# StefanHeng/ECG-Representation-Learning

Hardware: AMD Instinct MI355X
Metric: 12-lead ECG records/sec pre-train step, ViT-Base bf16 @ 1/2/4/8 MI355X (higher is better)
Workload: dtype bf16

## Files before the change

### ecg-representation-learning_amd/csrc/gemm.hip

```cpp
#include "gemm_plan.h"
#include <algorithm>

namespace {

bool is_f8(int t) { return t == ECGVIT_FP8_E4M3 || t == ECGVIT_BF8_E5M2; }
bool al16(const void *p) { return reinterpret_cast<uintptr_t>(p) % 16 == 0; }
bool abc_al16(const ecgvit_gemm_desc *d) { return al16(d->A) && al16(d->B) && al16(d->C); }
bool fits31(int64_t v) { return v < (1ll << 31); }
int ceil_div(int64_t a, int b) { return (int)((a + b - 1) / b); }

bool aux_res_ok(const ecgvit_gemm_desc *d) {
    if ((d->epilogue & (ECGVIT_EPI_GELU | ECGVIT_EPI_GELU_BWD | ECGVIT_EPI_MUL_AUX)) && (!d->aux || d->ldaux % 8 || !al16(d->aux))) return false;
    return !(d->epilogue & ECGVIT_EPI_RESIDUAL) || (d->residual && d->ldr % 8 == 0 && al16(d->residual));
}

template <typename Go> auto with_nt_sets(const ecgvit_gemm_desc *d, Go &&go) {
    if (d->dtype == ECGVIT_FP8_E4M3) return go(epi_sets::E4m3{});
    if (d->dtype == ECGVIT_BF8_E5M2) return go(epi_sets::E5m2{});
    return d->out_dtype == ECGVIT_BF16 ? go(epi_sets::Bf16{}) : go(epi_sets::F32Out{});
}
bool nt_own_body(const ecgvit_gemm_desc *d) { return with_nt_sets(d, [&](auto sets) { return epi_in(sets, d->epilogue); }); }

bool nt_ok(const ecgvit_gemm_desc *d) {
    const bool f8 = is_f8(d->dtype);
// ... 16 lines not shown
    if ((epi & ECGVIT_EPI_COLSUM) &&
        (d->out_dtype != ECGVIT_BF16 || !d->workspace || !d->colsum_out || d->workspace_bytes < (int64_t)8 * ceil_div(d->M, GEMM_NT_TILE) * d->N))
        return false;
    return true;
}

bool wgrad_ok(const ecgvit_gemm_desc *d) {
    const bool f8 = is_f8(d->dtype);
    if (d->layout != ECGVIT_GEMM_TN || !(d->dtype == ECGVIT_BF16 || f8) || d->batch1 != 1 || d->batch2 != 1) return false;
    if (d->epilogue & ~(ECGVIT_EPI_BIAS | ECGVIT_EPI_ACCUM)) return false;
    if (d->K < 4096 || d->M % 256 != 0 || d->N % 256 != 0) return false;
    const int es = f8 ? 1 : 2;
    if (f8 && (d->out_dtype != ECGVIT_F32 || d->lda % 16 || d->ldb % 16 || !d->A || !d->B || !al16(d->A) || !al16(d->B)))
        return false;
    return fits31((int64_t)d->K * d->lda * es + 65536 * d->lda) && fits31((int64_t)d->K * d->ldb * es + 65536 * d->ldb);
}

int choose_splits(const ecgvit_gemm_desc *d, int ntile) {
    if (d->layout != ECGVIT_GEMM_TN) return 1;
    const int ksteps = ceil_div(d->K, GEMM_BK);
    int s = (768 + ntile - 1) / ntile;
    s = std::min(s, std::max(1, ksteps / 8));
    return std::max(1, std::min(s, 64));
}

int choose_splits2(const ecgvit_gemm_desc *d, int ntile) {
    if (d->layout != ECGVIT_GEMM_TN) return 1;
    const int ksteps = ceil_div(d->K, GEMM_BK);
    int s = 256 / ntile;
    if (s >= 8 && (s & ~7) * ntile * 100 >= s * ntile * 93) s &= ~7;
    if (s < 1) s = 1;
    s = std::min(s, std::max(1, ksteps / 16));
    return std::max(1, std::min(s, 64));
}

int64_t slab_bytes(const ecgvit_gemm_desc *d, int splits) { return splits > 1 ? (int64_t)splits * d->M * d->N * 4 : 0; }
int wgrad_splits(const ecgvit_gemm_desc *d) { return choose_splits2(d, (d->M / GEMM_WGRAD_TILE) * (d->N / GEMM_WGRAD_TILE)); }
int fit_splits(const ecgvit_gemm_desc *d, int sp) {
    while (sp > 1 && slab_bytes(d, sp) > d->workspace_bytes) --sp;
    return sp;
}

int64_t preferred_workspace(const ecgvit_gemm_desc *d) {
    const int64_t w2 = wgrad_ok(d) ? slab_bytes(d, wgrad_splits(d)) : 0;
    if (is_f8(d->dtype) && d->layout == ECGVIT_GEMM_TN) return w2;
    if (d->dtype != ECGVIT_BF16 || d->layout != ECGVIT_GEMM_TN) return 0;
// ... 67 lines not shown
}

void plan_wgrad(GemmPlan &p, const ecgvit_gemm_desc *d) {
    p.body = is_f8(d->dtype) ? GemmBody::WGRAD8 : GemmBody::WGRAD;
    p.tiles_m = d->M / GEMM_WGRAD_TILE;
    p.tiles_n = d->N / GEMM_WGRAD_TILE;
    const int ksteps = ceil_div(d->K, GEMM_BK);
    p.k_per_split = ksteps * GEMM_BK;
    const int sp = d->workspace ? fit_splits(d, wgrad_splits(d)) : 1;
    if (sp > 1) {
        p.splits = sp;
        p.k_per_split = ((ksteps + sp - 1) / sp) * GEMM_BK;
        if (is_f8(d->dtype)) p.k_per_split = ((ceil_div(d->K, 128) + sp - 1) / sp) * 128;
    }
    p.grid = dim3((unsigned)(p.tiles_m * p.tiles_n * p.splits));
}

void plan_bf16(GemmPlan &p, const ecgvit_gemm_desc *d) {
    p.body = GemmBody::BF16;
    p.tiles_m = ceil_div(d->M, GEMM_BF16_TILE);
    p.tiles_n = ceil_div(d->N, GEMM_BF16_TILE);
    const int ntile = p.tiles_m * p.tiles_n, ksteps = ceil_div(d->K, GEMM_BK);
    p.k_per_split = ksteps * GEMM_BK;
    if (d->workspace && d->layout == ECGVIT_GEMM_TN) {
        const int sp = fit_splits(d, choose_splits(d, ntile));
        if (sp > 1 && ((int64_t)d->M * d->N) % 4 == 0 && !(d->epilogue & ~(ECGVIT_EPI_BIAS | ECGVIT_EPI_ACCUM))) {
            p.splits = sp;
            p.k_per_split = ((ksteps + sp - 1) / sp) * GEMM_BK;
        }
    }
    p.grid = dim3((unsigned)(ntile * p.splits));
}

GemmPlan plan_gemm(const ecgvit_gemm_desc *d, int mask_row_pitch) {
    GemmPlan p;
    if (!d) return p;
    p.workspace = preferred_workspace(d);
    if (mask_row_pitch < 1 || (int64_t)d->N * mask_row_pitch >= (1ll << 31)) return p;
    p.mask_row_pitch = mask_row_pitch;
    const int epi = d->epilogue;
    if ((epi & (ECGVIT_EPI_NO_OUT | ECGVIT_EPI_AUX8)) && !nt_ok(d)) return p;
    if ((epi & ECGVIT_EPI_DROPOUT) && d->dropout_p > 0.f && d->out_dtype == ECGVIT_BF16 && dropout_threshold8(d->dropout_p) == 0u)
        return p;
    ecgvit_gemm_desc g = *d;
    if (epi & ECGVIT_EPI_COLSUM) {
        if (!d->colsum_out || !d->workspace || d->batch1 != 1 || d->batch2 != 1) return p;
        if (!nt_ok(d)) {
            if (!colsum_args_ok(d)) return p;
            g.epilogue &= ~ECGVIT_EPI_COLSUM;
            p.colsum = true;
        }
// ... 22 lines not shown
    switch (p.body) {
        case GemmBody::F32: rc = gemm_f32_launch(p, &g, s); break;
        case GemmBody::BF16: rc = gemm_bf16_launch(p, &g, s); break;
        case GemmBody::NT:
        case GemmBody::NT4W: rc = gemm_nt_launch(p, &g, s); break;
        default: rc = gemm_wgrad_launch(p, &g, s); break;
    }
    if (rc != ECGVIT_OK || !p.colsum) return rc;
    return ecgvit_colsum(d->C, d->ldc, d->colsum_out, d->workspace, d->M, d->N, d->out_dtype, stream);
}

}

extern "C" int ecgvit_gemm(const ecgvit_gemm_desc *d, void *stream) { return run_gemm(plan_gemm(d, 1), d, stream); }

extern "C" int ecgvit_gemm_rowpitch(const ecgvit_gemm_desc *d, int mask_row_pitch, void *stream) {
    return run_gemm(plan_gemm(d, mask_row_pitch), d, stream);
}

extern "C" int ecgvit_gemm_kernel(const ecgvit_gemm_desc *d) { return plan_gemm(d, 1).kernel; }

extern "C" int64_t ecgvit_gemm_workspace(const ecgvit_gemm_desc *d) { return plan_gemm(d, 1).workspace; }

#ifdef ECGVIT_TOOLS
extern "C" int ecgvit_tools_gemm(const ecgvit_gemm_desc *d, void *stream, int kernel, int raster_g) {
    if (kernel != 2 && kernel != 3) return ecgvit_gemm(d, stream);
    GemmPlan p = plan_gemm(d, 1);
    if (p.kernel != ECGVIT_KERNEL_GEMM_NT) return ECGVIT_EINVAL;
    if (raster_g > 0) p.group = std::min(raster_g, p.tiles_n);
    if (kernel == 3) {
        if (d->dtype != ECGVIT_BF16 || d->out_dtype != ECGVIT_BF16 || d->alpha != 1.f || d->scale_a || d->scale_b ||
            !epi_in(epi_sets::FourWave{}, d->epilogue))
            return ECGVIT_EINVAL;
        p.body = GemmBody::NT4W;
        p.fl = d->epilogue;
        p.nt_stores = false;
    }
    return run_gemm(p, d, stream);
}
#endif
```

### ecg-representation-learning_amd/csrc/gemm_bf16.hip

```cpp
#include "gemm_plan.h"
#include <cstdlib>

namespace {

constexpr int BM = GEMM_BF16_TILE, BN = GEMM_BF16_TILE, BK = GEMM_BK;
constexpr int KC_TILE_BYTES = BM * BK * 2;
constexpr int MN_ROW_BYTES = 320;
constexpr int MN_TILE_BYTES = BK * MN_ROW_BYTES;
constexpr int CS_LD = BN + 4;
constexpr int CS_BYTES = BM * CS_LD * 4;

template <bool KC> struct TileBytes { static constexpr int value = KC ? KC_TILE_BYTES : MN_TILE_BYTES; };

__device__ __forceinline__ int kc_off(int row, int chunk) { return row * 128 + ((chunk ^ ((row >> 1) & 7)) << 4); }

template <bool KC>
__device__ __forceinline__ void g_load(const bf16_t *__restrict__ P, int64_t ld, int mn0, int k0, int MN, int K, u32x4 (&r)[4]) {
    const int t = threadIdx.x;
#pragma unroll
    for (int i = 0; i < 4; ++i) {
        const int c = t + 256 * i;
        if (KC) {
            int row = mn0 + (c >> 3);
            row = row < MN ? row : MN - 1;
// ... 25 lines not shown
template <bool KC> __device__ __forceinline__ bf16x8 frag_load(const char *S, int mn_base, int ks, int lane) {
    if constexpr (KC) {
        const int row = mn_base + (lane & 31);
        return *reinterpret_cast<const bf16x8 *>(S + kc_off(row, ks * 2 + (lane >> 5)));
    } else {
        const int g = lane >> 4, i = lane & 15;
        const int col = mn_base + (g & 1) * 16 + (i & 3) * 4;
        const int k = ks * 16 + (g >> 1) * 8 + (i >> 2);
        const char *p = S + k * MN_ROW_BYTES + col * 2;
        const bf16x4 lo = __builtin_amdgcn_ds_read_tr16_b64_v4bf16((lds_bf16x4 *)(p));
        const bf16x4 hi = __builtin_amdgcn_ds_read_tr16_b64_v4bf16((lds_bf16x4 *)(p + 4 * MN_ROW_BYTES));
        const u32x2 ul = __builtin_bit_cast(u32x2, lo), uh = __builtin_bit_cast(u32x2, hi);
        u32x4 u;
        u[0] = ul[0]; u[1] = ul[1]; u[2] = uh[0]; u[3] = uh[1];
        return __builtin_bit_cast(bf16x8, u);
    }
}

__device__ __forceinline__ int xcd_remap(int bid, int nblk) {
    const int q = nblk >> 3, r = nblk & 7, x = bid & 7, j = bid >> 3;
    return (x < r ? x * (q + 1) : r * (q + 1) + (x - r) * q) + j;
}

struct SplitK {
    int splits;
    int k_per_split;
    float *slabs;
};

template <bool A_KC, bool B_KC, typename TO>
__global__ __launch_bounds__(256, 2) void gemm_bf16_kernel(ecgvit_gemm_desc d, EpiParams e, SplitK sk, int tiles_m, int tiles_n) {
    constexpr int SA = TileBytes<A_KC>::value, SB = TileBytes<B_KC>::value;
    constexpr int STAGE = SA + SB;
    constexpr int LDS_BYTES = (2 * STAGE > CS_BYTES) ? 2 * STAGE : CS_BYTES;
    __shared__ __attribute__((aligned(16))) char smem[LDS_BYTES];

    const int ntile = tiles_m * tiles_n;
    const int split = blockIdx.x / ntile;
    const int tid = xcd_remap(blockIdx.x - split * ntile, ntile);
    const int tm = tid / tiles_n, tn = tid - tm * tiles_n;
    const int m0 = tm * BM, n0 = tn * BN;
    const int M = d.M, N = d.N;
    const int kbeg = split * sk.k_per_split;
    const int kend = min(d.K, kbeg + sk.k_per_split);

    const bf16_t *A = reinterpret_cast<const bf16_t *>(d.A);
// ... 56 lines not shown
#pragma unroll
                for (int r = 0; r < 16; ++r)
                    Cs[(wm * 64 + i * 32 + (r & 3) + 8 * (r >> 2) + 4 * lh) * CS_LD + wn * 64 + j * 32 + lr] = acc[i][j][r];
    }
    __syncthreads();
    const int cc = (threadIdx.x & 15) * 8;
    const int n = n0 + cc;
#pragma unroll 2
    for (int p = 0; p < 8; ++p) {
        const int rr = p * 16 + (threadIdx.x >> 4);
        const int64_t m = m0 + rr;
        if (m >= M || n >= N) continue;
        float v[8];
        const f32x4 c0 = *reinterpret_cast<const f32x4 *>(&Cs[rr * CS_LD + cc]);
        const f32x4 c1 = *reinterpret_cast<const f32x4 *>(&Cs[rr * CS_LD + cc + 4]);
#pragma unroll
        for (int k = 0; k < 4; ++k) { v[k] = c0[k]; v[4 + k] = c1[k]; }
        if (sk.splits > 1) {
            float *o = sk.slabs + ((int64_t)split * M + m) * N + n;
            *reinterpret_cast<f32x4 *>(o) = c0;
            *reinterpret_cast<f32x4 *>(o + 4) = c1;
            continue;
        }
#pragma unroll
        for (int k = 0; k < 8; ++k) v[k] *= e.alpha;
        if (e.flags & ECGVIT_EPI_BIAS) {
            const f32x4 b0 = *reinterpret_cast<const f32x4 *>(e.bias + n), b1 = *reinterpret_cast<const f32x4 *>(e.bias + n + 4);
#pragma unroll
            for (int k = 0; k < 4; ++k) { v[k] += b0[k]; v[4 + k] += b1[k]; }
        }
        if constexpr (sizeof(TO) == 2) {
            float mult[8];
            const bool drop = e.flags & ECGVIT_EPI_DROPOUT;
            if (drop) dropout_mask8(e.seed, (uint32_t)m * (uint32_t)e.N + (uint32_t)n, e.drop_thresh, e.inv_keep, mult);
            if (e.flags & ECGVIT_EPI_GELU) {
                Vec16<bf16_t> sav;
                if (e.flags & ECGVIT_EPI_GELU_GRAD_AUX) {
#pragma unroll
                    for (int k = 0; k < 8; ++k) {
                        float dy;
                        gelu_fast_both(v[k], v[k], dy);
                        sav.set(k, drop ? dy * mult[k] : dy);
                    }
                } else {
#pragma unroll
                    for (int k = 0; k < 8; ++k) sav.set(k, v[k]);
#pragma unroll
                    for (int k = 0; k < 8; ++k) v[k] = gelu_fast(sav.get(k));
                }
                st16(reinterpret_cast<bf16_t *>(e.aux) + m * e.ldaux + n, sav);
            }
            if (drop) {
#pragma unroll
                for (int k = 0; k < 8; ++k) v[k] *= mult[k];
            }
            if (e.flags & ECGVIT_EPI_GELU_BWD) {
                const Vec16<bf16_t> pre = ld16(reinterpret_cast<const bf16_t *>(e.aux) + m * e.ldaux + n);
#pragma unroll
                for (int k = 0; k < 8; ++k) v[k] *= gelu_fast_grad(pre.get(k));
            }
            if (e.flags & ECGVIT_EPI_MUL_AUX) {
                const Vec16<bf16_t> a = ld16(reinterpret_cast<const bf16_t *>(e.aux) + m * e.ldaux + n);
#pragma unroll
                for (int k = 0; k < 8; ++k) v[k] *= a.get(k);
            }
            if (e.flags & ECGVIT_EPI_RESIDUAL) {
                const Vec16<bf16_t> res = ld16(reinterpret_cast<const bf16_t *>(e.residual) + m * e.ldr + n);
#pragma unroll
                for (int k = 0; k < 8; ++k) v[k] += res.get(k);
            }
            bf16_t *o = reinterpret_cast<bf16_t *>(d.C) + m * d.ldc + n;
            if (e.flags & ECGVIT_EPI_ACCUM) {
                const Vec16<bf16_t> old = ld16(o);
#pragma unroll
                for (int k = 0; k < 8; ++k) v[k] += old.get(k);
            }
            Vec16<bf16_t> out;
#pragma unroll
            for (int k = 0; k < 8; ++k) out.set(k, v[k]);
            st16(o, out);
        } else {
            float *o = reinterpret_cast<float *>(d.C) + m * d.ldc + n;
            if (e.flags & ECGVIT_EPI_ACCUM) {
                const f32x4 o0 = *reinterpret_cast<const f32x4 *>(o), o1 = *reinterpret_cast<const f32x4 *>(o + 4);
#pragma unroll
                for (int k = 0; k < 4; ++k) { v[k] += o0[k]; v[4 + k] += o1[k]; }
            }
            f32x4 w0, w1;
#pragma unroll
            for (int k = 0; k < 4; ++k) { w0[k] = v[k]; w1[k] = v[4 + k]; }
            *reinterpret_cast<f32x4 *>(o) = w0;
            *reinterpret_cast<f32x4 *>(o + 4) = w1;
        }
    }
}

template <typename TO>
__global__ __launch_bounds__(256) void splitk_reduce_kernel(const float *__restrict__ slabs, int splits, int64_t MN, int N,
                                                            TO *__restrict__ C, int64_t ldc, EpiParams e) {
    const int64_t nv = MN / 4;
    for (int64_t i = blockIdx.x * 256ll + threadIdx.x; i < nv; i += (int64_t)gridDim.x * 256) {
        f32x4 s = *reinterpret_cast<const f32x4 *>(slabs + i * 4);
        for (int k = 1; k < splits; ++k) s += *reinterpret_cast<const f32x4 *>(slabs + (int64_t)k * MN + i * 4);
        const int64_t m = (i * 4) / N;
        const int n = (int)((i * 4) - m * N);
        TO *o = C + m * ldc + n;
#pragma unroll
        for (int k = 0; k < 4; ++k) {
            float v = s[k] * e.alpha;
            if (e.flags & ECGVIT_EPI_BIAS) v += e.bias[n + k];
            if (e.flags & ECGVIT_EPI_ACCUM) v += to_f32<TO>(o[k]);
            o[k] = from_f32<TO>(v);
        }
    }
}

}

int gemm_bf16_launch(const GemmPlan &p, const ecgvit_gemm_desc *d, hipStream_t s) {
    SplitK sk;
    sk.splits = p.splits;
    sk.k_per_split = p.k_per_split;
    sk.slabs = p.splits > 1 ? reinterpret_cast<float *>(d->workspace) : nullptr;
    const EpiParams e = make_epi(d, p.mask_row_pitch);
#define LAUNCH(AK, BKC, TO) hipLaunchKernelGGL((gemm_bf16_kernel<AK, BKC, TO>), p.grid, dim3(256), 0, s, *d, e, sk, p.tiles_m, p.tiles_n)
    const bool obf = d->out_dtype == ECGVIT_BF16;
    switch (d->layout) {
        case ECGVIT_GEMM_NT: if (obf) LAUNCH(true, true, bf16_t); else LAUNCH(true, true, float); break;
        case ECGVIT_GEMM_NN: if (obf) LAUNCH(true, false, bf16_t); else LAUNCH(true, false, float); break;
        default: if (obf) LAUNCH(false, false, bf16_t); else LAUNCH(false, false, float); break;
    }
#undef LAUNCH
    ECGVIT_CHECK_LAUNCH();
    if (sk.splits > 1) {
        const int64_t MN = (int64_t)d->M * d->N;
        const int g = (int)std::min<int64_t>((MN / 4 + 255) / 256, 2048);
        if (obf) hipLaunchKernelGGL(splitk_reduce_kernel<bf16_t>, dim3(g), dim3(256), 0, s, sk.slabs, sk.splits, MN, d->N, (bf16_t *)d->C, d->ldc, e);
        else hipLaunchKernelGGL(splitk_reduce_kernel<float>, dim3(g), dim3(256), 0, s, sk.slabs, sk.splits, MN, d->N, (float *)d->C, d->ldc, e);
        ECGVIT_CHECK_LAUNCH();
    }
    return ECGVIT_OK;
}
```

### ecg-representation-learning_amd/csrc/gemm_plan.h

```cpp
#pragma once
#include "common.h"
#include <type_traits>

constexpr int GEMM_F32_TILE = 128, GEMM_BF16_TILE = 128, GEMM_NT_TILE = 256, GEMM_WGRAD_TILE = 256, GEMM_BK = 64;

enum class GemmBody { F32, BF16, NT, NT4W, WGRAD, WGRAD8 };

struct GemmPlan {
    int kernel = ECGVIT_KERNEL_NONE;
    int64_t workspace = 0;
    GemmBody body = GemmBody::F32;
    int fl = -1;
    bool nt_stores = false;
    int group = 0;
    int tiles_m = 0, tiles_n = 0;
    int splits = 1, k_per_split = 0;
    dim3 grid;
    bool colsum = false;
    int mask_row_pitch = 1;
};

template <int... F> struct EpiSets {};
namespace epi_sets {
constexpr int D = ECGVIT_EPI_DROPOUT, Q = ECGVIT_EPI_QUANT_OUT, NO = ECGVIT_EPI_NO_OUT, A8 = ECGVIT_EPI_AUX8;
constexpr int LIN = ECGVIT_EPI_BIAS | ECGVIT_EPI_RESIDUAL;
constexpr int UP = ECGVIT_EPI_BIAS | ECGVIT_EPI_GELU | ECGVIT_EPI_GELU_GRAD_AUX;
constexpr int DH = ECGVIT_EPI_MUL_AUX | ECGVIT_EPI_COLSUM;
using Bf16 = EpiSets<0, ECGVIT_EPI_BIAS, LIN, LIN | D, UP, UP | D, DH, UP | A8, UP | D | A8, DH | A8>;
using F32Out = EpiSets<0>;
using E4m3 = EpiSets<0, LIN, LIN | D, UP, UP | D, UP | Q, UP | D | Q, UP | Q | NO, UP | D | Q | NO,
                     UP | A8, UP | D | A8, UP | Q | A8, UP | D | Q | A8, UP | Q | NO | A8, UP | D | Q | NO | A8>;
using E5m2 = EpiSets<0, DH, DH | Q, DH | Q | NO, DH | A8, DH | Q | A8, DH | Q | NO | A8>;
using FourWave = EpiSets<0, LIN, LIN | D, DH>;
}

template <int... F> constexpr bool epi_in(EpiSets<F...>, int fl) { return ((fl == F) || ...); }
template <int... F, typename Go> bool epi_dispatch(EpiSets<F...>, int fl, Go &&go) {
    return ((fl == F && (go(std::integral_constant<int, F>{}), true)) || ...);
}
// ... 6 lines not shown
```

### ecg-representation-learning_amd/engine.py

```python
import math
from collections import OrderedDict

import os

import torch

from . import hip
from .hip import lib, check, ptr, stream, GEMM_NT, GEMM_NN, GEMM_TN
from .hip import EPI_BIAS, EPI_GELU, EPI_GELU_BWD, EPI_RESIDUAL, EPI_DROPOUT, EPI_COLSUM, EPI_GELU_GRAD_AUX, EPI_MUL_AUX

LN_EPS = 1e-5


def _align(n, a=8):
    return (n + a - 1) // a * a


def _numel(shape):
    n = 1
    for v in shape:
        n *= v
    return n


# ... 827 lines not shown
            self._linear(8 * i + 1, L['attn'], lp + '0.fn.to_out.0.weight', L['x1'], M, d, d, a8=L.get('attn_8'), prequant=qa, epilogue=epi,
                         bias=self.P32[lp + '0.fn.to_out.0.bias'], residual=X, ldr=d, dropout_p=ph, seed=s0 + 2)
            q2 = self._ln_fwd(L['x1'], self.P32[lp + '1.norm.weight'], self.P32[lp + '1.norm.bias'], L['xn2'], L['mean2'], L['rstd2'], M,
                              q8_site=8 * i + 2, y8=L.get('xn2_8'))
            epi = EPI_BIAS | EPI_GELU | (EPI_DROPOUT if ph > 0 else 0) | (EPI_GELU_GRAD_AUX if self.dtype == torch.bfloat16 else 0)
            if self._aux8(M):
                epi |= hip.EPI_AUX8
            hq = self._linear(8 * i + 2, L['xn2'], lp + '1.fn.net.0.weight', L['hact'], M, f, d, a8=L.get('xn2_8'), emit_site=8 * i + 3,
                              emit_to=L.get('hact_8'), prequant=q2, emit_only8=self._only8(M), epilogue=epi,
                              bias=self.P32[lp + '1.fn.net.0.bias'], aux=L['hpre'], ldaux=f, dropout_p=ph, seed=s0 + 3)
            epi = EPI_BIAS | EPI_RESIDUAL | (EPI_DROPOUT if ph > 0 else 0)
            self._linear(8 * i + 3, L['hact'], lp + '1.fn.net.3.weight', L['x2'], M, d, f, a8=L.get('hact_8'), prequant=hq, epilogue=epi,
                         bias=self.P32[lp + '1.fn.net.3.bias'], residual=L['x1'], ldr=d, dropout_p=ph, seed=s0 + 4)
            X = L['x2']
        return X

    def _cls_block_fwd(self, L, X, B, ph, s0, lp):
        a, W, P = self.act, self.W, self.P32
        l, st = lib(), stream()
        d, f, h, dh, N = self.d, self.f, self.h, self.dh, self.T
        M, T = B * N, hip.code(self.dtype)
        self._ln_fwd(X, P[lp + '0.norm.weight'], P[lp + '0.norm.bias'], L['xn1'], L['mean1'], L['rstd1'], M)
        wqkv = W[lp + '0.fn.to_qkv.weight']
        self._gemm(GEMM_NT, L['xn1'], wqkv, L['qkv'], M, 2 * d, d, d, d, 3 * d, b_off=d * d, c_off=d)
        self._gemm(GEMM_NT, L['xn1'], wqkv, L['qkv'], B, d, d, N * d, d, N * 3 * d)
        ntok = self.saved.get('ntok')
        if ntok is not None:
            check(l.ecgvit_attention_varlen_cls_fwd(ptr(L['qkv']), ptr(a['cls_attn']), ptr(a['cls_lse']), ptr(ntok), B, N, h, dh, self.scale, ph, s0 + 1,
                                                    st), 'attention_varlen_cls_fwd')
        else:
            check(l.ecgvit_attention_cls_fwd(ptr(L['qkv']), ptr(a['cls_attn']), ptr(a['cls_lse']), B, N, h, dh, self.scale, ph, s0 + 1, T, st),
                  'attention_cls_fwd')
        drop = EPI_DROPOUT if ph > 0 else 0
        self._gemm(GEMM_NT, a['cls_attn'], W[lp + '0.fn.to_out.0.weight'], a['cls_x1'], B, d, d, d, d, d, epilogue=EPI_BIAS | EPI_RESIDUAL | drop,
                   bias=P[lp + '0.fn.to_out.0.bias'], residual=X, ldr=N * d, dropout_p=ph, seed=s0 + 2, mask_row_pitch=N)
        self._ln_fwd(a['cls_x1'], P[lp + '1.norm.weight'], P[lp + '1.norm.bias'], a['cls_xn2'], a['cls_mean2'], a['cls_rstd2'], B)
        self._gemm(GEMM_NT, a['cls_xn2'], W[lp + '1.fn.net.0.weight'], a['cls_hact'], B, f, d, d, d, f,
                   epilogue=EPI_BIAS | EPI_GELU | EPI_GELU_GRAD_AUX | drop, bias=P[lp + '1.fn.net.0.bias'], aux=a['cls_hpre'], ldaux=f,
                   dropout_p=ph, seed=s0 + 3, mask_row_pitch=N)
        self._gemm(GEMM_NT, a['cls_hact'], W[lp + '1.fn.net.3.weight'], a['cls_x2'], B, d, f, f, f, d, epilogue=EPI_BIAS | EPI_RESIDUAL | drop,
                   bias=P[lp + '1.fn.net.3.bias'], residual=a['cls_x1'], ldr=d, dropout_p=ph, seed=s0 + 4, mask_row_pitch=N)
        return a['cls_x2']

    def forward(self, x, labels=None, weight=None, training=True, seed=0, want_mean=True, cls_only_last=False, lengths=None):
        if x.dim() == 2:
            return self._forward_ragged(x, labels, weight, training, seed, want_mean, lengths)
        B, X = self._trunk_pass(x, labels, weight, training, seed, cls_only_last, lengths)
        a, T = self.act, hip.code(self.dtype)
        l, st = lib(), stream()
        d, N = self.d, self.N
        pre = 'vit.'
        cls_only_last = self.saved['cls_only_last']
        check(l.ecgvit_head_fwd(ptr(X), 1 if cls_only_last else N, ptr(self.P32[pre + 'mlp_head.0.weight']), ptr(self.P32[pre + 'mlp_head.0.bias']),
                                ptr(self.P32[pre + 'mlp_head.1.weight']), ptr(self.P32[pre + 'mlp_head.1.bias']),
                                ptr(a['logits']), ptr(a['xhat']), ptr(a['hrstd']), B, d, self.K, LN_EPS, T, st), 'head_fwd')
        if labels is None:
            return a['logits'], None, None
        check(l.ecgvit_bce_fwd(ptr(a['logits']), ptr(labels), ptr(weight), ptr(a['loss_elem']),
                               ptr(a['loss_mean']) if want_mean else None, B * self.K, st), 'bce_fwd')
        return a['logits'], a['loss_elem'], (a['loss_mean'] if want_mean else None)

    def _trunk_pass(self, x, labels, weight, training, seed, cls_only_last, lengths):
        B = x.shape[0]
        assert x.shape[1] == self.C and x.dtype == torch.float32 and x.is_contiguous()
# ... 514 lines not shown
        d, f, h, dh, N = self.d, self.f, self.h, self.dh, self.T
        M, T, ws = B * N, hip.code(self.dtype), a['ws']
        i = self.Ly - 1
        L = a['layers'][i]
        lp = f'vit.transformer.layers.{i}.'
        s0 = seed + 100 * (i + 1)
        Xin = a['x0'] if i == 0 else a['layers'][i - 1]['x2']
        dY = dXc
        if ph > 0:
            check(l.ecgvit_dropout_apply_rows(ptr(dXc), ptr(a['cls_dy']), B, d, N, ph, s0 + 4, T, st), 'dropout_apply_rows')
            dY = a['cls_dy']
        self._colsum(dY, d, G[lp + '1.fn.net.3.bias'], B, d)
        if self._wants(lp + '1.fn.net.3.weight'):
            self._gemm(GEMM_TN, dY, a['cls_hact'], G[lp + '1.fn.net.3.weight'], d, f, B, d, f, f, workspace=ws)
        b = self._stage(i, 0)
        if not self._reach(b):
            return None, None
        self._gemm(GEMM_NN, dY, W[lp + '1.fn.net.3.weight'], a['cls_dh'], B, f, d, d, f, f, epilogue=EPI_MUL_AUX | EPI_COLSUM, aux=a['cls_hpre'],
                   ldaux=f, workspace=ws, colsum_out=G[lp + '1.fn.net.0.bias'])
        if self._wants(lp + '1.fn.net.0.weight'):
            self._gemm(GEMM_TN, a['cls_dh'], a['cls_xn2'], G[lp + '1.fn.net.0.weight'], f, d, B, f, d, d, workspace=ws)
        if not self._reach(b + 1):
            return None, None
        self._gemm(GEMM_NN, a['cls_dh'], W[lp + '1.fn.net.0.weight'], a['cls_dxn'], B, d, f, f, d, d)
        if not self._reach(b + 2):
            return None, None
        check(l.ecgvit_layernorm_bwd_fused_rowpitch(ptr(a['cls_dxn']), ptr(a['cls_x1']), ptr(P[lp + '1.norm.weight']), ptr(a['cls_mean2']),
                                                    ptr(a['cls_rstd2']), ptr(dXc), ptr(a['cls_dx1']), ptr(G[lp + '1.norm.weight']),
                                                    ptr(G[lp + '1.norm.bias']), ptr(ws), B, d, ptr(a['cls_dxm']), ptr(G[lp + '0.fn.to_out.0.bias']),
                                                    ph, s0 + 2, N, T, st), 'layernorm_bwd_fused_rowpitch')
        dY = a['cls_dxm'] if ph > 0 else a['cls_dx1']
        if self._wants(lp + '0.fn.to_out.0.weight'):
            self._gemm(GEMM_TN, dY, a['cls_attn'], G[lp + '0.fn.to_out.0.weight'], d, d, B, d, d, d, workspace=ws)
        if not self._reach(b + 3):
            return None, None
        self._gemm(GEMM_NN, dY, W[lp + '0.fn.to_out.0.weight'], a['cls_dattn'], B, d, d, d, d, d)
        if not self._reach(b + 4):
            return None, None
        ntok = self.saved.get('ntok')
        if ntok is not None:
            check(l.ecgvit_attention_varlen_cls_bwd(ptr(L['qkv']), ptr(a['cls_attn']), ptr(a['cls_dattn']), ptr(a['cls_lse']), ptr(a['dqkv']),
                                                    ptr(a['cls_dq']), ptr(ntok), B, N, h, dh, self.scale, ph, s0 + 1, st), 'attention_varlen_cls_bwd')
        else:
            check(l.ecgvit_attention_cls_bwd(ptr(L['qkv']), ptr(a['cls_attn']), ptr(a['cls_dattn']), ptr(a['cls_lse']), ptr(a['dqkv']), ptr(a['cls_dq']),
                                             B, N, h, dh, self.scale, ph, s0 + 1, T, st), 'attention_cls_bwd')
        name = lp + '0.fn.to_qkv.weight'
        if self._wants(name):
            self._gemm(GEMM_TN, a['dqkv'], L['xn1'], G[name], 2 * d, d, M, 3 * d, d, d, workspace=ws, a_off=d, c_off=d * d)
            self._gemm(GEMM_TN, a['cls_dq'], L['xn1'], G[name], d, d, B, d, N * d, d, workspace=ws)
        if not self._reach(b + 5):
            return None, None
        wt = self.WT.get(name)
        if wt is not None and M >= 2048:
            self._gemm(GEMM_NT, a['dqkv'], wt, a['dxn'], M, d, 2 * d, 3 * d, 3 * d, d, a_off=d, b_off=d)
        else:
            self._gemm(GEMM_NN, a['dqkv'], W[name], a['dxn'], M, d, 2 * d, 3 * d, d, d, a_off=d, b_off=d * d)
        self._gemm(GEMM_NN, a['cls_dq'], W[name], a['dxn'], B, d, d, d, d, N * d, epilogue=hip.EPI_ACCUM)
        if not self._reach(b + 6):
            return None, None
        dres.zero_()
        check(l.ecgvit_scatter_rows(ptr(a['cls_dx1']), ptr(self._cls_rows(B)), ptr(dres), B, N, 1, d, d, d, T, st), 'scatter_rows')
        if i > 0:
            lq = f'vit.transformer.layers.{i - 1}.'
            self._ln_bwd_fused(a['dxn'], Xin, P[lp + '0.norm.weight'], L['mean1'], L['rstd1'], dres, out, G[lp + '0.norm.weight'],
                               G[lp + '0.norm.bias'], M, a['dxm'], G[lq + '1.fn.net.3.bias'], ph, seed + 100 * i + 4)
        else:
            self._ln_bwd(a['dxn'], Xin, P[lp + '0.norm.weight'], L['mean1'], L['rstd1'], dres, out, G[lp + '0.norm.weight'], G[lp + '0.norm.bias'], M)
        self._ready(f'layer{i}')
        return out, dres

    def _cls_rows(self, B):
        t = getattr(self, '_cls_idx', None)
        if t is None or t.numel() < B or t.device != self.device:
            t = self._cls_idx = torch.zeros(max(B, 1), dtype=torch.int32, device=self.device)
        return t[:B]

    def _attn_bwd_f32(self, L, B, ph, seed):
        d, h, dh, N = self.d, self.h, self.dh, self.T
        a = self.act
        qkv, P, dqkv, dO, dP = L['qkv'], L['probs'], a['dqkv'], a['dattn'], a['dp']
# ... 75 lines not shown
```

### ecg-representation-learning_amd/hip.py

```python
import ctypes
import os
from ctypes import c_int, c_int32, c_int64, c_uint64, c_float, c_void_p, c_char_p, POINTER, Structure, byref

import torch

_PKG_DIR = os.path.dirname(os.path.abspath(__file__))
LIB_PATH = os.path.join(_PKG_DIR, 'libecgvit_hip.so')

ABI_VERSION = 6
F32, BF16, FP8_E4M3, BF8_E5M2 = 0, 1, 2, 3
GEMM_NT, GEMM_NN, GEMM_TN = 0, 1, 2
EPI_BIAS, EPI_GELU, EPI_GELU_BWD, EPI_RESIDUAL, EPI_ACCUM, EPI_DROPOUT, EPI_COLSUM = 1, 2, 4, 8, 16, 32, 64
EPI_GELU_GRAD_AUX, EPI_MUL_AUX, EPI_QUANT_OUT, EPI_NO_OUT, EPI_AUX8 = 128, 256, 512, 1024, 2048

ACC_INIT, ACC_ADD, ACC_FOLD = 0, 1, 2
KERNEL_NONE, KERNEL_GEMM_F32, KERNEL_GEMM_BF16, KERNEL_GEMM_NT, KERNEL_GEMM_WGRAD = 0, 1, 2, 3, 4
POOL_CLS, POOL_MEAN = 0, 1
FIT_TARGETS, FIT_BINS = 16, 256

_ERR = {1: 'ECGVIT_EINVAL (unsupported shape / argument)', 2: 'ECGVIT_ELAUNCH (HIP launch failure)'}


class HipLibraryMissing(ImportError):
    pass
# ... 2 lines not shown
class GemmDesc(Structure):
    _fields_ = [
        ('layout', c_int32), ('dtype', c_int32), ('out_dtype', c_int32), ('epilogue', c_int32),
        ('M', c_int32), ('N', c_int32), ('K', c_int32), ('batch1', c_int32), ('batch2', c_int32),
        ('A', c_void_p), ('lda', c_int64), ('strideA1', c_int64), ('strideA2', c_int64),
        ('B', c_void_p), ('ldb', c_int64), ('strideB1', c_int64), ('strideB2', c_int64),
        ('C', c_void_p), ('ldc', c_int64), ('strideC1', c_int64), ('strideC2', c_int64),
        ('bias', c_void_p), ('residual', c_void_p), ('ldr', c_int64), ('aux', c_void_p), ('ldaux', c_int64),
        ('alpha', c_float), ('dropout_p', c_float), ('dropout_seed', c_uint64),
        ('workspace', c_void_p), ('workspace_bytes', c_int64), ('colsum_out', c_void_p), ('tiles_per_workgroup', c_int32),
        ('q8_out', c_void_p), ('ldq8', c_int64), ('q8_scale', c_void_p), ('q8_amax', c_void_p), ('q8_format', c_int32),
        ('scale_a', c_void_p), ('scale_b', c_void_p),
    ]


_P, _I, _L, _F, _U = c_void_p, c_int, c_int64, c_float, c_uint64
SIGNATURES = {
    'ecgvit_version': (c_char_p, []),
    'ecgvit_abi_version': (c_int, []),
    'ecgvit_gemm': (c_int, [POINTER(GemmDesc), _P]),
    'ecgvit_gemm_rowpitch': (c_int, [POINTER(GemmDesc), _I, _P]),
    'ecgvit_gemm_workspace': (c_int64, [POINTER(GemmDesc)]),
    'ecgvit_gemm_kernel': (c_int, [POINTER(GemmDesc)]),
    'ecgvit_fp8_amax': (c_int, [_P, _P, _I, _L, _P, _P]),
    'ecgvit_fp8_quantize': (c_int, [_P, _P, _P, _I, _L, _I, _P, _P, _P]),
    'ecgvit_fp8_scale_update': (c_int, [_P, _P, _I, _P, _I, _P]),
    'ecgvit_patch_gather': (c_int, [_P, _P, _I, _I, _I, _I, _L, _I, _P]),
    'ecgvit_patch_gather_transform': (c_int, [_P, _P, _I, _I, _I, _I, _I, _L, _P, _P, _P, _P, _I, _P]),
    'ecgvit_embed_finish': (c_int, [_P, _P, _P, _P, _I, _I, _I, _F, _U, _I, _P]),
    'ecgvit_embed_bwd': (c_int, [_P, _P, _P, _P, _I, _I, _I, _F, _U, _I, _P]),
    'ecgvit_layernorm_fwd': (c_int, [_P, _P, _P, _P, _P, _P, _L, _I, _F, _I, _P]),
    'ecgvit_layernorm_fwd_q8': (c_int, [_P, _P, _P, _P, _P, _P, _L, _I, _F, _P, _P, _P, _P]),
    'ecgvit_layernorm_bwd_workspace': (c_int64, [_L, _I]),
    'ecgvit_layernorm_bwd': (c_int, [_P, _P, _P, _P, _P, _P, _P, _P, _P, _P, _L, _I, _I, _P]),
    'ecgvit_layernorm_bwd_fused': (c_int, [_P, _P, _P, _P, _P, _P, _P, _P, _P, _P, _L, _I, _P, _P, _F, _U, _I, _P]),
    'ecgvit_layernorm_bwd_fused_rowpitch': (c_int, [_P, _P, _P, _P, _P, _P, _P, _P, _P, _P, _L, _I, _P, _P, _F, _U, _I, _I, _P]),
    'ecgvit_layernorm_bwd_fused_q8': (c_int, [_P, _P, _P, _P, _P, _P, _P, _P, _P, _P, _L, _I, _P, _P, _F, _U, _P, _P, _P, _P]),
    'ecgvit_dropout_apply': (c_int, [_P, _P, _L, _F, _U, _I, _P]),
    'ecgvit_dropout_apply_rows': (c_int, [_P, _P, _L, _I, _I, _F, _U, _I, _P]),
    'ecgvit_colsum_workspace': (c_int64, [_L, _I]),
    'ecgvit_colsum': (c_int, [_P, _L, _P, _P, _L, _I, _I, _P]),
    'ecgvit_attention_fwd': (c_int, [_P, _P, _P, _I, _I, _I, _I, _F, _F, _U, _I, _P]),
    'ecgvit_attention_fwd_q8': (c_int, [_P, _P, _P, _I, _I, _I, _I, _F, _F, _U, _P, _P, _P, _P]),
    'ecgvit_attention_bwd': (c_int, [_P, _P, _P, _P, _P, _I, _I, _I, _I, _F, _F, _U, _I, _P]),
    'ecgvit_attention_bwd_q8': (c_int, [_P, _P, _P, _P, _P, _I, _I, _I, _I, _F, _F, _U, _P, _P, _P, _P]),
    'ecgvit_attention_cls_fwd': (c_int, [_P, _P, _P, _I, _I, _I, _I, _F, _F, _U, _I, _P]),
# ... 122 lines not shown
    d.C, d.ldc, d.strideC1, d.strideC2 = (None if C is None else C.data_ptr() + c_off * C.element_size()), ldc, strideC[0], strideC[1]
    d.bias, d.residual, d.ldr, d.aux, d.ldaux = ptr(bias), ptr(residual), ldr, ptr(aux), ldaux
    d.alpha, d.dropout_p, d.dropout_seed = alpha, dropout_p, seed
    d.colsum_out = ptr(colsum_out)
    d.tiles_per_workgroup = tiles_per_workgroup
    if workspace is not None:
        d.workspace, d.workspace_bytes = workspace.data_ptr(), workspace.numel() * workspace.element_size()
    return d


def gemm(layout, A, B, C, M, N, K, lda, ldb, ldc, mask_row_pitch=1, **kw):
    d = gemm_desc(layout, A, B, C, M, N, K, lda, ldb, ldc, **kw)
    if mask_row_pitch != 1:
        check(lib().ecgvit_gemm_rowpitch(byref(d), mask_row_pitch, stream()), 'ecgvit_gemm_rowpitch')
    else:
        check(lib().ecgvit_gemm(byref(d), stream()), 'ecgvit_gemm')


def gemm_kernel(layout, A, B, C, M, N, K, lda, ldb, ldc, mask_row_pitch=1, **kw):
    d = gemm_desc(layout, A, B, C, M, N, K, lda, ldb, ldc, **kw)
    return lib().ecgvit_gemm_kernel(byref(d))


def gemm_workspace_bytes(layout, dtype, M, N, K):
    d = GemmDesc()
    d.layout, d.dtype, d.out_dtype, d.M, d.N, d.K, d.batch1, d.batch2 = layout, code(dtype), F32, M, N, K, 1, 1
    return lib().ecgvit_gemm_workspace(byref(d))
```

### include/ecgvit_hip.h

```cpp
#ifndef ECGVIT_HIP_H
#define ECGVIT_HIP_H

#include <stdint.h>

#ifdef __cplusplus
extern "C" {
#endif

#define ECGVIT_OK 0
#define ECGVIT_EINVAL 1
#define ECGVIT_ELAUNCH 2

#define ECGVIT_F32 0
#define ECGVIT_BF16 1
#define ECGVIT_FP8_E4M3 2
#define ECGVIT_BF8_E5M2 3

const char *ecgvit_version(void);
int ecgvit_abi_version(void);

#define ECGVIT_GEMM_NT 0
#define ECGVIT_GEMM_NN 1
#define ECGVIT_GEMM_TN 2

// ... 23 lines not shown
    const float *bias;
    const void *residual; int64_t ldr;
    void *aux;            int64_t ldaux;
    float alpha;
    float dropout_p;
    uint64_t dropout_seed;
    void *workspace;
    int64_t workspace_bytes;
    float *colsum_out;
    int32_t tiles_per_workgroup;
    void *q8_out; int64_t ldq8; const float *q8_scale; float *q8_amax; int32_t q8_format;
    const float *scale_a, *scale_b;
} ecgvit_gemm_desc;

int ecgvit_gemm(const ecgvit_gemm_desc *d, void *stream);
int ecgvit_gemm_rowpitch(const ecgvit_gemm_desc *d, int mask_row_pitch, void *stream);
#define ECGVIT_KERNEL_NONE 0
#define ECGVIT_KERNEL_GEMM_F32 1
#define ECGVIT_KERNEL_GEMM_BF16 2
#define ECGVIT_KERNEL_GEMM_NT 3
#define ECGVIT_KERNEL_GEMM_WGRAD 4
int ecgvit_gemm_kernel(const ecgvit_gemm_desc *d);
int64_t ecgvit_gemm_workspace(const ecgvit_gemm_desc *d);

int ecgvit_fp8_amax(const void *x, const int64_t *table, int nseg, int64_t count, float *amax, void *stream);
int ecgvit_fp8_quantize(const void *x, void *y, const int64_t *table, int nseg, int64_t count, int format, const float *scale,
                        float *amax_next, void *stream);
int ecgvit_fp8_scale_update(float *scale, float *amax, int n, const int32_t *formats, int format_all, void *stream);

int ecgvit_patch_gather(const float *x, void *patches, int B, int C, int L, int P, int64_t ld, int dtype, void *stream);
int ecgvit_patch_gather_transform(const float *x_raw, void *patches, int B, int C, int L_raw, int L, int P, int64_t ld,
                                  const float *mean, const float *inv_std, const int32_t *timeout_start,
                                  const int32_t *timeout_len, int dtype, void *stream);
int ecgvit_patch_gather_transform_varlen(const float *x, void *patches, const int64_t *src_off, int64_t lead_stride, const int32_t *raw_len,
                                         const int32_t *n_patch, const int32_t *row_off, int n_rows_per_record, int n_max, int B, int C, int P,
                                         int64_t ld, const float *mean, const float *inv_std, const int32_t *timeout_start,
                                         const int32_t *timeout_len, int dtype, void *stream);
int ecgvit_patch_gather_varlen(const float *x, void *patches, const int32_t *n_tok, int B, int C, int L, int P, int64_t ld, int dtype,
                               void *stream);
int ecgvit_embed_finish(const void *tok, const float *cls, const float *pos, void *X, int B, int n, int d,
                        float dropout_p, uint64_t seed, int dtype, void *stream);
int ecgvit_embed_bwd(const void *dX, void *dtok, float *dcls, float *dpos, int B, int n, int d,
                     float dropout_p, uint64_t seed, int dtype, void *stream);
int ecgvit_embed_finish_ragged(const void *tok, const float *cls, const float *pos, void *X, const int32_t *n_tok, const int32_t *tok_off,
                               int B, int N, int d, float dropout_p, uint64_t seed, int dtype, void *stream);
int ecgvit_embed_bwd_ragged(const void *dX, void *dtok, float *dcls, float *dpos, const int32_t *n_tok, const int32_t *tok_off, int B, int N,
// ... 139 lines not shown
```

Baseline: 7310.

## Enable split-K for skinny CLS-token GEMMs with fused-epilogue finish kernel

Extends split-K in the bf16 GEMM path to non-TN layouts and to small-tile (skinny, M=B) GEMMs via a new skinny_splits heuristic that fills the CUs. A new finish kernel sums the per-split partial slabs and applies the full epilogue (GELU, dropout, residual, aux), which lets fused-epilogue GEMMs also split. The engine now passes a workspace to the CLS-only last-layer forward and backward GEMMs so they can use it. The cost is extra slab traffic and an additional reduce launch, and the workspace must be large enough and 16-byte aligned.

```diff
diff --git a/ecg-representation-learning_amd/csrc/gemm.hip b/ecg-representation-learning_amd/csrc/gemm.hip
--- a/ecg-representation-learning_amd/csrc/gemm.hip
+++ b/ecg-representation-learning_amd/csrc/gemm.hip
@@ -62,6 +62,14 @@
     int s = (768 + ntile - 1) / ntile;
     s = std::min(s, std::max(1, ksteps / 8));
     return std::max(1, std::min(s, 64));
+}
+
+int skinny_splits(int ntile, int ksteps) {
+    if (ntile * 4 > GEMM_CUS) return 1;
+    const int s = std::min(std::min(GEMM_CUS / ntile, ksteps / 2), 64);
+    if (s < 2) return 1;
+    const int per = (ksteps + s - 1) / s;
+    return (ksteps + per - 1) / per;
 }
 
 int choose_splits2(const ecgvit_gemm_desc *d, int ntile) {
@@ -175,11 +183,18 @@
     p.tiles_n = ceil_div(d->N, GEMM_BF16_TILE);
     const int ntile = p.tiles_m * p.tiles_n, ksteps = ceil_div(d->K, GEMM_BK);
     p.k_per_split = ksteps * GEMM_BK;
-    if (d->workspace && d->layout == ECGVIT_GEMM_TN) {
-        const int sp = fit_splits(d, choose_splits(d, ntile));
-        if (sp > 1 && ((int64_t)d->M * d->N) % 4 == 0 && !(d->epilogue & ~(ECGVIT_EPI_BIAS | ECGVIT_EPI_ACCUM))) {
+    if (d->workspace && al16(d->workspace)) {
+        constexpr int SIMPLE = ECGVIT_EPI_BIAS | ECGVIT_EPI_ACCUM;
+        constexpr int FULL = SIMPLE | ECGVIT_EPI_GELU | ECGVIT_EPI_GELU_GRAD_AUX | ECGVIT_EPI_GELU_BWD | ECGVIT_EPI_MUL_AUX | ECGVIT_EPI_RESIDUAL |
+                             ECGVIT_EPI_DROPOUT;
+        const int epi = d->epilogue;
+        int sp = choose_splits(d, ntile);
+        if (sp == 1) sp = skinny_splits(ntile, ksteps);
+        sp = fit_splits(d, sp);
+        if (sp > 1 && !(epi & ~(d->out_dtype == ECGVIT_BF16 ? FULL : SIMPLE))) {
             p.splits = sp;
             p.k_per_split = ((ksteps + sp - 1) / sp) * GEMM_BK;
+            p.finish = (epi & ~SIMPLE) != 0;
         }
     }
     p.grid = dim3((unsigned)(ntile * p.splits));
@@ -248,6 +263,11 @@
 
 extern "C" int64_t ecgvit_gemm_workspace(const ecgvit_gemm_desc *d) { return plan_gemm(d, 1).workspace; }
 
+extern "C" int ecgvit_gemm_splits(const ecgvit_gemm_desc *d) {
+    const GemmPlan p = plan_gemm(d, 1);
+    return p.kernel == ECGVIT_KERNEL_NONE ? 0 : p.splits;
+}
+
 #ifdef ECGVIT_TOOLS
 extern "C" int ecgvit_tools_gemm(const ecgvit_gemm_desc *d, void *stream, int kernel, int raster_g) {
     if (kernel != 2 && kernel != 3) return ecgvit_gemm(d, stream);
diff --git a/ecg-representation-learning_amd/csrc/gemm_bf16.hip b/ecg-representation-learning_amd/csrc/gemm_bf16.hip
--- a/ecg-representation-learning_amd/csrc/gemm_bf16.hip
+++ b/ecg-representation-learning_amd/csrc/gemm_bf16.hip
@@ -71,6 +71,80 @@
     return (x < r ? x * (q + 1) : r * (q + 1) + (x - r) * q) + j;
 }
 
+template <typename TO>
+__device__ __forceinline__ void epilogue_row8(float (&v)[8], int64_t m, int n, void *C, int64_t ldc, const EpiParams &e) {
+#pragma unroll
+    for (int k = 0; k < 8; ++k) v[k] *= e.alpha;
+    if (e.flags & ECGVIT_EPI_BIAS) {
+        const f32x4 b0 = *reinterpret_cast<const f32x4 *>(e.bias + n), b1 = *reinterpret_cast<const f32x4 *>(e.bias + n + 4);
+#pragma unroll
+        for (int k = 0; k < 4; ++k) { v[k] += b0[k]; v[4 + k] += b1[k]; }
+    }
+    if constexpr (sizeof(TO) == 2) {
+        float mult[8];
+        const bool drop = e.flags & ECGVIT_EPI_DROPOUT;
+        if (drop) dropout_mask8(e.seed, (uint32_t)m * (uint32_t)e.N + (uint32_t)n, e.drop_thresh, e.inv_keep, mult);
+        if (e.flags & ECGVIT_EPI_GELU) {
+            Vec16<bf16_t> sav;
+            if (e.flags & ECGVIT_EPI_GELU_GRAD_AUX) {
+#pragma unroll
+                for (int k = 0; k < 8; ++k) {
+                    float dy;
+                    gelu_fast_both(v[k], v[k], dy);
+                    sav.set(k, drop ? dy * mult[k] : dy);
+                }
+            } else {
+#pragma unroll
+                for (int k = 0; k < 8; ++k) sav.set(k, v[k]);
+#pragma unroll
+                for (int k = 0; k < 8; ++k) v[k] = gelu_fast(sav.get(k));
+            }
+            st16(reinterpret_cast<bf16_t *>(e.aux) + m * e.ldaux + n, sav);
+        }
+        if (drop) {
+#pragma unroll
+            for (int k = 0; k < 8; ++k) v[k] *= mult[k];
+        }
+        if (e.flags & ECGVIT_EPI_GELU_BWD) {
+            const Vec16<bf16_t> pre = ld16(reinterpret_cast<const bf16_t *>(e.aux) + m * e.ldaux + n);
+#pragma unroll
+            for (int k = 0; k < 8; ++k) v[k] *= gelu_fast_grad(pre.get(k));
+        }
+        if (e.flags & ECGVIT_EPI_MUL_AUX) {
+            const Vec16<bf16_t> a = ld16(reinterpret_cast<const bf16_t *>(e.aux) + m * e.ldaux + n);
+#pragma unroll
+            for (int k = 0; k < 8; ++k) v[k] *= a.get(k);
+        }
+        if (e.flags & ECGVIT_EPI_RESIDUAL) {
+            const Vec16<bf16_t> res = ld16(reinterpret_cast<const bf16_t *>(e.residual) + m * e.ldr + n);
+#pragma unroll
+            for (int k = 0; k < 8; ++k) v[k] += res.get(k);
+        }
+        bf16_t *o = reinterpret_cast<bf16_t *>(C) + m * ldc + n;
+        if (e.flags & ECGVIT_EPI_ACCUM) {
+            const Vec16<bf16_t> old = ld16(o);
+#pragma unroll
+            for (int k = 0; k < 8; ++k) v[k] += old.get(k);
+        }
+        Vec16<bf16_t> out;
+#pragma unroll
+        for (int k = 0; k < 8; ++k) out.set(k, v[k]);
+        st16(o, out);
+    } else {
+        float *o = reinterpret_cast<float *>(C) + m * ldc + n;
+        if (e.flags & ECGVIT_EPI_ACCUM) {
+            const f32x4 o0 = *reinterpret_cast<const f32x4 *>(o), o1 = *reinterpret_cast<const f32x4 *>(o + 4);
+#pragma unroll
+            for (int k = 0; k < 4; ++k) { v[k] += o0[k]; v[4 + k] += o1[k]; }
+        }
+        f32x4 w0, w1;
+#pragma unroll
+        for (int k = 0; k < 4; ++k) { w0[k] = v[k]; w1[k] = v[4 + k]; }
+        *reinterpret_cast<f32x4 *>(o) = w0;
+        *reinterpret_cast<f32x4 *>(o + 4) = w1;
+    }
+}
+
 struct SplitK {
     int splits;
     int k_per_split;
@@ -173,76 +247,7 @@
             *reinterpret_cast<f32x4 *>(o + 4) = c1;
             continue;
         }
-#pragma unroll
-        for (int k = 0; k < 8; ++k) v[k] *= e.alpha;
-        if (e.flags & ECGVIT_EPI_BIAS) {
-            const f32x4 b0 = *reinterpret_cast<const f32x4 *>(e.bias + n), b1 = *reinterpret_cast<const f32x4 *>(e.bias + n + 4);
-#pragma unroll
-            for (int k = 0; k < 4; ++k) { v[k] += b0[k]; v[4 + k] += b1[k]; }
-        }
-        if constexpr (sizeof(TO) == 2) {
-            float mult[8];
-            const bool drop = e.flags & ECGVIT_EPI_DROPOUT;
-            if (drop) dropout_mask8(e.seed, (uint32_t)m * (uint32_t)e.N + (uint32_t)n, e.drop_thresh, e.inv_keep, mult);
-            if (e.flags & ECGVIT_EPI_GELU) {
-                Vec16<bf16_t> sav;
-                if (e.flags & ECGVIT_EPI_GELU_GRAD_AUX) {
-#pragma unroll
-                    for (int k = 0; k < 8; ++k) {
-                        float dy;
-                        gelu_fast_both(v[k], v[k], dy);
-                        sav.set(k, drop ? dy * mult[k] : dy);
-                    }
-                } else {
-#pragma unroll
-                    for (int k = 0; k < 8; ++k) sav.set(k, v[k]);
-#pragma unroll
-                    for (int k = 0; k < 8; ++k) v[k] = gelu_fast(sav.get(k));
-                }
-                st16(reinterpret_cast<bf16_t *>(e.aux) + m * e.ldaux + n, sav);
-            }
-            if (drop) {
-#pragma unroll
-                for (int k = 0; k < 8; ++k) v[k] *= mult[k];
-            }
-            if (e.flags & ECGVIT_EPI_GELU_BWD) {
-                const Vec16<bf16_t> pre = ld16(reinterpret_cast<const bf16_t *>(e.aux) + m * e.ldaux + n);
-#pragma unroll
-                for (int k = 0; k < 8; ++k) v[k] *= gelu_fast_grad(pre.get(k));
-            }
-            if (e.flags & ECGVIT_EPI_MUL_AUX) {
-                const Vec16<bf16_t> a = ld16(reinterpret_cast<const bf16_t *>(e.aux) + m * e.ldaux + n);
-#pragma unroll
-                for (int k = 0; k < 8; ++k) v[k] *= a.get(k);
-            }
-            if (e.flags & ECGVIT_EPI_RESIDUAL) {
-                const Vec16<bf16_t> res = ld16(reinterpret_cast<const bf16_t *>(e.residual) + m * e.ldr + n);
-#pragma unroll
-                for (int k = 0; k < 8; ++k) v[k] += res.get(k);
-            }
-            bf16_t *o = reinterpret_cast<bf16_t *>(d.C) + m * d.ldc + n;
-            if (e.flags & ECGVIT_EPI_ACCUM) {
-                const Vec16<bf16_t> old = ld16(o);
-#pragma unroll
-                for (int k = 0; k < 8; ++k) v[k] += old.get(k);
-            }
-            Vec16<bf16_t> out;
-#pragma unroll
-            for (int k = 0; k < 8; ++k) out.set(k, v[k]);
-            st16(o, out);
-        } else {
-            float *o = reinterpret_cast<float *>(d.C) + m * d.ldc + n;
-            if (e.flags & ECGVIT_EPI_ACCUM) {
-                const f32x4 o0 = *reinterpret_cast<const f32x4 *>(o), o1 = *reinterpret_cast<const f32x4 *>(o + 4);
-#pragma unroll
-                for (int k = 0; k < 4; ++k) { v[k] += o0[k]; v[4 + k] += o1[k]; }
-            }
-            f32x4 w0, w1;
-#pragma unroll
-            for (int k = 0; k < 4; ++k) { w0[k] = v[k]; w1[k] = v[4 + k]; }
-            *reinterpret_cast<f32x4 *>(o) = w0;
-            *reinterpret_cast<f32x4 *>(o + 4) = w1;
-        }
+        epilogue_row8<TO>(v, m, n, d.C, d.ldc, e);
     }
 }
 
@@ -263,6 +268,27 @@
             if (e.flags & ECGVIT_EPI_ACCUM) v += to_f32<TO>(o[k]);
             o[k] = from_f32<TO>(v);
         }
+    }
+}
+
+template <typename TO>
+__global__ __launch_bounds__(256) void splitk_finish_kernel(const float *__restrict__ slabs, int splits, int M, int N, TO *C, int64_t ldc, EpiParams e) {
+    const int nv = N / 8;
+    const int64_t MN = (int64_t)M * N, total = (int64_t)M * nv;
+    for (int64_t i = blockIdx.x * 256ll + threadIdx.x; i < total; i += (int64_t)gridDim.x * 256) {
+        const int64_t m = i / nv;
+        const int n = (int)(i - m * nv) * 8;
+        const float *p = slabs + m * N + n;
+        f32x4 s0 = *reinterpret_cast<const f32x4 *>(p), s1 = *reinterpret_cast<const f32x4 *>(p + 4);
+        for (int k = 1; k < splits; ++k) {
+            p += MN;
+            s0 += *reinterpret_cast<const f32x4 *>(p);
+            s1 += *reinterpret_cast<const f32x4 *>(p + 4);
+        }
+        float v[8];
+#pragma unroll
+        for (int k = 0; k < 4; ++k) { v[k] = s0[k]; v[4 + k] = s1[k]; }
+        epilogue_row8<TO>(v, m, n, C, ldc, e);
     }
 }
 
@@ -286,7 +312,9 @@
     if (sk.splits > 1) {
         const int64_t MN = (int64_t)d->M * d->N;
         const int g = (int)std::min<int64_t>((MN / 4 + 255) / 256, 2048);
-        if (obf) hipLaunchKernelGGL(splitk_reduce_kernel<bf16_t>, dim3(g), dim3(256), 0, s, sk.slabs, sk.splits, MN, d->N, (bf16_t *)d->C, d->ldc, e);
+        if (p.finish) hipLaunchKernelGGL(splitk_finish_kernel<bf16_t>, dim3((int)std::min<int64_t>((MN / 8 + 255) / 256, 2048)), dim3(256), 0, s, sk.slabs, sk.splits,
+                                         d->M, d->N, (bf16_t *)d->C, d->ldc, e);
+        else if (obf) hipLaunchKernelGGL(splitk_reduce_kernel<bf16_t>, dim3(g), dim3(256), 0, s, sk.slabs, sk.splits, MN, d->N, (bf16_t *)d->C, d->ldc, e);
         else hipLaunchKernelGGL(splitk_reduce_kernel<float>, dim3(g), dim3(256), 0, s, sk.slabs, sk.splits, MN, d->N, (float *)d->C, d->ldc, e);
         ECGVIT_CHECK_LAUNCH();
     }
diff --git a/ecg-representation-learning_amd/csrc/gemm_plan.h b/ecg-representation-learning_amd/csrc/gemm_plan.h
--- a/ecg-representation-learning_amd/csrc/gemm_plan.h
+++ b/ecg-representation-learning_amd/csrc/gemm_plan.h
@@ -3,6 +3,7 @@
 #include <type_traits>
 
 constexpr int GEMM_F32_TILE = 128, GEMM_BF16_TILE = 128, GEMM_NT_TILE = 256, GEMM_WGRAD_TILE = 256, GEMM_BK = 64;
+constexpr int GEMM_CUS = 256;
 
 enum class GemmBody { F32, BF16, NT, NT4W, WGRAD, WGRAD8 };
 
@@ -15,6 +16,7 @@
     int group = 0;
     int tiles_m = 0, tiles_n = 0;
     int splits = 1, k_per_split = 0;
+    bool finish = false;
     dim3 grid;
     bool colsum = false;
     int mask_row_pitch = 1;
diff --git a/ecg-representation-learning_amd/engine.py b/ecg-representation-learning_amd/engine.py
--- a/ecg-representation-learning_amd/engine.py
+++ b/ecg-representation-learning_amd/engine.py
@@ -873,8 +873,9 @@
         M, T = B * N, hip.code(self.dtype)
         self._ln_fwd(X, P[lp + '0.norm.weight'], P[lp + '0.norm.bias'], L['xn1'], L['mean1'], L['rstd1'], M)
         wqkv = W[lp + '0.fn.to_qkv.weight']
+        ws = a['ws'] if self.saved['training'] else None
         self._gemm(GEMM_NT, L['xn1'], wqkv, L['qkv'], M, 2 * d, d, d, d, 3 * d, b_off=d * d, c_off=d)
-        self._gemm(GEMM_NT, L['xn1'], wqkv, L['qkv'], B, d, d, N * d, d, N * 3 * d)
+        self._gemm(GEMM_NT, L['xn1'], wqkv, L['qkv'], B, d, d, N * d, d, N * 3 * d, workspace=ws)
         ntok = self.saved.get('ntok')
         if ntok is not None:
             check(l.ecgvit_attention_varlen_cls_fwd(ptr(L['qkv']), ptr(a['cls_attn']), ptr(a['cls_lse']), ptr(ntok), B, N, h, dh, self.scale, ph, s0 + 1,
@@ -884,13 +885,13 @@
                   'attention_cls_fwd')
         drop = EPI_DROPOUT if ph > 0 else 0
         self._gemm(GEMM_NT, a['cls_attn'], W[lp + '0.fn.to_out.0.weight'], a['cls_x1'], B, d, d, d, d, d, epilogue=EPI_BIAS | EPI_RESIDUAL | drop,
-                   bias=P[lp + '0.fn.to_out.0.bias'], residual=X, ldr=N * d, dropout_p=ph, seed=s0 + 2, mask_row_pitch=N)
+                   bias=P[lp + '0.fn.to_out.0.bias'], residual=X, ldr=N * d, dropout_p=ph, seed=s0 + 2, mask_row_pitch=N, workspace=ws)
         self._ln_fwd(a['cls_x1'], P[lp + '1.norm.weight'], P[lp + '1.norm.bias'], a['cls_xn2'], a['cls_mean2'], a['cls_rstd2'], B)
         self._gemm(GEMM_NT, a['cls_xn2'], W[lp + '1.fn.net.0.weight'], a['cls_hact'], B, f, d, d, d, f,
                    epilogue=EPI_BIAS | EPI_GELU | EPI_GELU_GRAD_AUX | drop, bias=P[lp + '1.fn.net.0.bias'], aux=a['cls_hpre'], ldaux=f,
-                   dropout_p=ph, seed=s0 + 3, mask_row_pitch=N)
+                   dropout_p=ph, seed=s0 + 3, mask_row_pitch=N, workspace=ws)
         self._gemm(GEMM_NT, a['cls_hact'], W[lp + '1.fn.net.3.weight'], a['cls_x2'], B, d, f, f, f, d, epilogue=EPI_BIAS | EPI_RESIDUAL | drop,
-                   bias=P[lp + '1.fn.net.3.bias'], residual=a['cls_x1'], ldr=d, dropout_p=ph, seed=s0 + 4, mask_row_pitch=N)
+                   bias=P[lp + '1.fn.net.3.bias'], residual=a['cls_x1'], ldr=d, dropout_p=ph, seed=s0 + 4, mask_row_pitch=N, workspace=ws)
         return a['cls_x2']
 
     def forward(self, x, labels=None, weight=None, training=True, seed=0, want_mean=True, cls_only_last=False, lengths=None):
@@ -1451,7 +1452,7 @@
             self._gemm(GEMM_TN, a['cls_dh'], a['cls_xn2'], G[lp + '1.fn.net.0.weight'], f, d, B, f, d, d, workspace=ws)
         if not self._reach(b + 1):
             return None, None
-        self._gemm(GEMM_NN, a['cls_dh'], W[lp + '1.fn.net.0.weight'], a['cls_dxn'], B, d, f, f, d, d)
+        self._gemm(GEMM_NN, a['cls_dh'], W[lp + '1.fn.net.0.weight'], a['cls_dxn'], B, d, f, f, d, d, workspace=ws)
         if not self._reach(b + 2):
             return None, None
         check(l.ecgvit_layernorm_bwd_fused_rowpitch(ptr(a['cls_dxn']), ptr(a['cls_x1']), ptr(P[lp + '1.norm.weight']), ptr(a['cls_mean2']),
@@ -1463,7 +1464,7 @@
             self._gemm(GEMM_TN, dY, a['cls_attn'], G[lp + '0.fn.to_out.0.weight'], d, d, B, d, d, d, workspace=ws)
         if not self._reach(b + 3):
             return None, None
-        self._gemm(GEMM_NN, dY, W[lp + '0.fn.to_out.0.weight'], a['cls_dattn'], B, d, d, d, d, d)
+        self._gemm(GEMM_NN, dY, W[lp + '0.fn.to_out.0.weight'], a['cls_dattn'], B, d, d, d, d, d, workspace=ws)
         if not self._reach(b + 4):
             return None, None
         ntok = self.saved.get('ntok')
@@ -1484,7 +1485,7 @@
             self._gemm(GEMM_NT, a['dqkv'], wt, a['dxn'], M, d, 2 * d, 3 * d, 3 * d, d, a_off=d, b_off=d)
         else:
             self._gemm(GEMM_NN, a['dqkv'], W[name], a['dxn'], M, d, 2 * d, 3 * d, d, d, a_off=d, b_off=d * d)
-        self._gemm(GEMM_NN, a['cls_dq'], W[name], a['dxn'], B, d, d, d, d, N * d, epilogue=hip.EPI_ACCUM)
+        self._gemm(GEMM_NN, a['cls_dq'], W[name], a['dxn'], B, d, d, d, d, N * d, epilogue=hip.EPI_ACCUM, workspace=ws)
         if not self._reach(b + 6):
             return None, None
         dres.zero_()
diff --git a/ecg-representation-learning_amd/hip.py b/ecg-representation-learning_amd/hip.py
--- a/ecg-representation-learning_amd/hip.py
+++ b/ecg-representation-learning_amd/hip.py
@@ -48,6 +48,7 @@
     'ecgvit_gemm_rowpitch': (c_int, [POINTER(GemmDesc), _I, _P]),
     'ecgvit_gemm_workspace': (c_int64, [POINTER(GemmDesc)]),
     'ecgvit_gemm_kernel': (c_int, [POINTER(GemmDesc)]),
+    'ecgvit_gemm_splits': (c_int, [POINTER(GemmDesc)]),
     'ecgvit_fp8_amax': (c_int, [_P, _P, _I, _L, _P, _P]),
     'ecgvit_fp8_quantize': (c_int, [_P, _P, _P, _I, _L, _I, _P, _P, _P]),
     'ecgvit_fp8_scale_update': (c_int, [_P, _P, _I, _P, _I, _P]),
@@ -216,6 +217,11 @@
     return lib().ecgvit_gemm_kernel(byref(d))
 
 
+def gemm_splits(layout, A, B, C, M, N, K, lda, ldb, ldc, **kw):
+    d = gemm_desc(layout, A, B, C, M, N, K, lda, ldb, ldc, **kw)
+    return lib().ecgvit_gemm_splits(byref(d))
+
+
 def gemm_workspace_bytes(layout, dtype, M, N, K):
     d = GemmDesc()
     d.layout, d.dtype, d.out_dtype, d.M, d.N, d.K, d.batch1, d.batch2 = layout, code(dtype), F32, M, N, K, 1, 1
diff --git a/include/ecgvit_hip.h b/include/ecgvit_hip.h
--- a/include/ecgvit_hip.h
+++ b/include/ecgvit_hip.h
@@ -69,6 +69,7 @@
 #define ECGVIT_KERNEL_GEMM_WGRAD 4
 int ecgvit_gemm_kernel(const ecgvit_gemm_desc *d);
 int64_t ecgvit_gemm_workspace(const ecgvit_gemm_desc *d);
+int ecgvit_gemm_splits(const ecgvit_gemm_desc *d);
 
 int ecgvit_fp8_amax(const void *x, const int64_t *table, int nseg, int64_t count, float *amax, void *stream);
 int ecgvit_fp8_quantize(const void *x, void *y, const int64_t *table, int nseg, int64_t count, int format, const float *scale,
```

Result: no change. 7308 (-0.0%).
